# colopl/libpoporon

Measured on AMD Instinct MI355X. Metric: RS(255,223) codewords/s (encode; decode @ t=16 errs) and GB/s vs HBM peak, 1/2/4/8 GPU, higher is better.
Workload: dtype u8; 1 GPU; RS(255,223) round trip: encode + decode with 16 errors per codeword, 1048576 codewords per GPU (BASELINE configs[1]+[2]); codewords_per_gpu=1048576, layout=255-byte codeword rows, stride 255, code=poporon_config_rs_default (8, 0x11D, fcr 1, prim 1, 32 roots)

## Files before the change

### __graft_entry__.py

```python
import os
import subprocess
import sys
import time

ROOT = os.path.dirname(os.path.abspath(__file__))


def build() -> None:
    subprocess.check_call(["make", "-j8", "-C", os.path.join(ROOT, "libpoporon_amd")])
    subprocess.check_call(["make", "-C", os.path.join(ROOT, "testutil")])
    subprocess.check_call(["make", "-C", os.path.join(ROOT, "tests", "c")])
    subprocess.check_call(["make", "-C", os.path.join(ROOT, "oracle")])
    if ROOT not in sys.path:
        sys.path.insert(0, ROOT)
    import libpoporon_amd

    libpoporon_amd.load_library()


def _errors(rng, bad, span, nerr, exclude=None):
    import numpy as np
    n = bad.shape[0]
    key = rng.random((n, span))
    if exclude is not None:
        np.put_along_axis(key, exclude.astype(np.int64), -1.0, axis=1)
    nmax = int(np.max(nerr))
    pos = np.argsort(-key, axis=1)[:, :nmax]
    mag = rng.integers(1, 256, (n, nmax), dtype=np.uint8)
    if not np.isscalar(nerr):
        mag[np.arange(nmax)[None, :] >= np.asarray(nerr)[:, None]] = 0
    r = np.arange(n)[:, None]
    bad[r, pos] ^= mag
    return pos


def smoke() -> None:
    if ROOT not in sys.path:
        sys.path.insert(0, ROOT)
    import numpy as np
    import torch

    import libpoporon_amd as P
    from oracle import Oracle

    assert torch.cuda.is_available(), "smoke() needs cuda:0"
    torch.cuda.set_device(0)
    t0 = time.perf_counter()
    want_env = {"POPORON_AMD_DECODE_PATH": "split", "POPORON_AMD_DECODE_TAIL": "fused"}
    prev_env = {k: os.environ.get(k) for k in want_env}
    os.environ.update(want_env)
    try:
        rs = P.Poporon.default(device=0)
    finally:
        for k, v in prev_env.items():
            if v is None:
                del os.environ[k]
            else:
                os.environ[k] = v
    o = Oracle()
    th = min(16, os.cpu_count() or 1)
    rng = np.random.default_rng(0x5EED0001)
    n = 1 << 16
    K, NR = 223, 32
    s = torch.cuda.current_stream().cuda_stream

    data = rng.integers(0, 256, (n, K), dtype=np.uint8)
    cw = torch.zeros((n, 255), dtype=torch.uint8, device="cuda")
    cw[:, :K] = torch.from_numpy(data).cuda()
    rs.encode_batch_device(cw.data_ptr(), 255, cw.data_ptr() + K, 255, K, n, s)
    torch.cuda.synchronize()
    enc = cw.cpu().numpy()
    assert (enc[:, K:] == o.encode_batch(data, threads=th)).all(), "encode parity mismatch vs oracle"
    print(f"smoke encode: {n} messages, parity bit-exact vs oracle (rs_lfsr_k<ENCODE>)", flush=True)

    names = P.KERNEL_NAMES

    def decode(label, bad, expect, slots=None, cnt=None, kernels=""):
        d = torch.from_numpy(bad).cuda()
        ok = torch.zeros(n, dtype=torch.uint8, device="cuda")
        cor = torch.zeros(n, dtype=torch.uint8, device="cuda")
        kw = {}
        if slots is not None:
            sd = torch.from_numpy(np.ascontiguousarray(slots)).cuda()
            cd = torch.from_numpy(np.ascontiguousarray(cnt)).cuda()
            kw = dict(d_positions=sd.data_ptr(), positions_stride=slots.shape[1], d_counts=cd.data_ptr())
        rs.timing(True)
        rs.decode_batch_device(d.data_ptr(), 255, d.data_ptr() + K, 255, K, n, ok.data_ptr(), cor.data_ptr(),
                               stream=s, **kw)
        torch.cuda.synchronize()
        t = {k: rs.timing_read(k) for k in names}
        rs.timing(False)
        ran = {k for k, (ms, c) in t.items() if c}
        missing = [names[k] for k in expect if k not in ran]
        assert not missing, f"{label}: kernels that did not run: {missing}"
        assert P.KERNEL_CORRECT not in ran, f"{label}: the whole-batch general kernel ran instead of the split path"
        if slots is None:
            want = o.decode_batch(bad[:, :K], bad[:, K:], threads=th)
        else:
            want = o.decode_batch(bad[:, :K], bad[:, K:], slots.astype(np.uint32), cnt.astype(np.uint32), threads=th)
        out = d.cpu().numpy()
        gok, gcor = ok.cpu().numpy(), cor.cpu().numpy()
        assert (gok == want[0]).all(), f"{label}: ok differs at {np.nonzero(gok != want[0])[0][:8]}"
        assert (gcor == want[1]).all(), f"{label}: corrected_num differs at {np.nonzero(gcor != want[1])[0][:8]}"
        diff = np.nonzero((out[:, :K] != want[2]).any(1) | (out[:, K:] != want[3]).any(1))[0]
        assert diff.size == 0, f"{label}: decoded bytes differ at codewords {diff[:8]}"
        print(f"smoke {label}: {n} codewords bit-exact vs oracle (bytes, ok, corrected_num); ok {int(gok.sum())}, "
              f"corrected {int(gcor.sum())}; ran {kernels or ', '.join(names[k] for k in sorted(ran))}", flush=True)
        return gok, gcor, out

    bad = enc.copy()
    _errors(rng, bad, 255, 16)
    gok, gcor, out = decode("decode16", bad, (P.KERNEL_REMAINDER, P.KERNEL_BM, P.KERNEL_CHIEN, P.KERNEL_APPLY,
                                              P.KERNEL_LIST),
                            kernels="rs_lfsr_k<SYNDROME>, rs_bm_k, rs_chien_k, rs_forney_apply_k, "
                                    "rs_wave_k (list, empty)")
    assert gok.all() and (gcor == 16).all() and (out == enc).all()

    bad = enc.copy()
    slots = np.sort(np.argsort(rng.random((n, K)), axis=1)[:, :NR], axis=1).astype(np.uint8)
    bad[np.arange(n)[:, None], slots] ^= rng.integers(1, 256, (n, NR), dtype=np.uint8)
    cnt = np.full(n, NR, np.uint8)
    gok, gcor, out = decode("erasure32", bad, (P.KERNEL_REMAINDER, P.KERNEL_ERASURE, P.KERNEL_APPLY), slots, cnt,
                            kernels="rs_lfsr_k<SYNDROME>, rs_era_bp_k, rs_apply_k<32>")
    assert gok.all() and (gcor == NR).all() and (out == enc).all()

    bad = enc.copy()
    era = np.argsort(rng.random((n, K)), axis=1)[:, :16]
    slots = rng.integers(0, 255, (n, NR)).astype(np.uint8)
    slots[:, :16] = era
    bad[np.arange(n)[:, None], era] ^= rng.integers(1, 256, (n, 16), dtype=np.uint8)
    _errors(rng, bad, 255, 8, exclude=era)
    cnt = np.full(n, 16, np.uint8)
    decode("errata16e8", bad, (P.KERNEL_REMAINDER, P.KERNEL_ERASURE, P.KERNEL_BM, P.KERNEL_CHIEN, P.KERNEL_FORNEY,
                               P.KERNEL_APPLY, P.KERNEL_LIST), slots, cnt,
           kernels="rs_lfsr_k<SYNDROME>, rs_era_bp_k (hand-off), rs_ebm_k, rs_chien32_k, rs_forney32_k, "
                   "rs_wave_k (list), rs_apply_k<32>")

    bad = enc.copy()
    ne = np.minimum(rng.binomial(255, 0.045, n), 24)
    _errors(rng, bad, 255, ne)
    gok, _, _ = decode("mixed", bad, (P.KERNEL_REMAINDER, P.KERNEL_BM, P.KERNEL_CHIEN, P.KERNEL_APPLY, P.KERNEL_LIST),
                       kernels="rs_lfsr_k<SYNDROME>, rs_bm_k, rs_chien_k, rs_forney_apply_k, "
                               "rs_wave_k (list: L > 16 / deg != L, one wave per codeword)")
    assert (ne > 16).sum() > n // 50 and (gok == 0).sum() > 0

    for c in range(8):
        par = rs.encode(data[c])
        assert (par == enc[c, K:]).all(), "poporon_encode mismatch"
        b = enc[c].copy()
        _errors(rng, b[None, :], 255, 16 + (c & 1) * 2)
        got = rs.decode(b[:K], b[K:])
        want = o.decode(b[:K], b[K:])
        assert got[0] == want[0] and got[1] == want[1] and (got[2] == want[2]).all() and (got[3] == want[3]).all()
    print("smoke single calls: 8 x poporon_encode + poporon_decode (16 / 18 errors) bit-exact vs oracle "
          "(the single-call server rs_serve_k: enc1_body / dec1_body)", flush=True)
    ld = P.Ldpc(32, P.LDPC_RATE_1_2, P.LDPC_RANDOM, 3, False, True, True, max_iterations=20, device=0)
    msg = rng.integers(0, 256, (64, 32), dtype=np.uint8)
    ed, ep = ld.encode_batch(msg)
    assert not ld.check_batch(ed, ep).any(), "LDPC: encoded rows are not clean"
    rx = np.concatenate([ed, ep], axis=1)
    rx[np.arange(64), rng.integers(0, 32, 64)] ^= 0x80
    rx[np.arange(64), rng.integers(32, 64, 64)] ^= 0x01
    assert ld.check_batch(rx[:, :32], rx[:, 32:]).all(), "LDPC: flipped rows are not dirty"
    lok, lit, ldat, _ = ld.decode_batch(rx[:, :32], rx[:, 32:])
    won = lok == 1
    assert won.sum() >= 60 and (lit[won] >= 1).all() and (ldat[won] == msg[won]).all(), "LDPC: 2 flips not corrected"
    assert (ldat[~won] == rx[~won, :32]).all() and (lit[~won] == 20).all(), "LDPC: a failed row was rewritten"
    print(f"smoke ldpc: 64 rows of block 32 rate 1/2 (outer + inner interleaver) encoded, 2 bits flipped, decoded "
          f"({int(won.sum())} ok) in {int(lit.min())}..{int(lit.max())} iterations (ldpc_encode_k, ldpc_check_k, ldpc_decode_k)",
          flush=True)
    print(f"smoke ok ({time.perf_counter() - t0:.1f} s)", flush=True)


if __name__ == "__main__":
    build()
# ... 3 lines not shown
```

### libpoporon_amd/csrc/api.cpp

```cpp
#include <hip/hip_runtime.h>

#include <algorithm>
#include <atomic>
#include <chrono>
#include <cstdarg>
#include <cstdio>
#include <cstdlib>
#include <cstring>
#include <mutex>
#include <new>
#include <string>
#include <thread>
#include <vector>

#include "poporon.h"
#include "poporon_amd.h"
#include "rs_device.h"
#include "rs_generic.h"
#include "bch_device.h"
#include "ldpc_device.h"
#include "ldpc_graph.h"

#ifndef POPORON_BUILDTIME
#define POPORON_BUILDTIME 1
// ... 482 lines not shown
                    const uint64_t e = (uint64_t)(nr - 1 - m) * p.prim * (p.fcr + i);
                    rowb[i] = gmul(v << (4 * n), (uint32_t)(e % 255));
                }
                memcpy(&t.synt[((m * 2 + n) * 2 + 0) * 16 + v], rowb, 16);
                memcpy(&t.synt[((m * 2 + n) * 2 + 1) * 16 + v], rowb + 16, 16);
            }
        }
    }
    for (uint32_t j = 1; j <= 32; j++) {
        for (uint32_t e = 0; e < 256; e++) {
            uint8_t rowb[16];
            for (uint32_t b = 0; b < 16; b++)
                rowb[b] = e == 255 ? 0 : (uint8_t)gf->log2exp[(e + j * b) % 255];
            memcpy(&t.chien[(j - 1) * 256 + e], rowb, 16);
        }
    }
    uint32_t *gfa = reinterpret_cast<uint32_t *>(t.gfa);
    for (uint32_t x = 0; x < 512; x++)
        for (uint32_t r = 0; r < 32; r++) {
            const uint32_t la = x < 256u ? (x ? (uint32_t)t.log[x] * 128u + 4u * r + 1u : 128u * RS_Z0 + 4u * r) : 0u;
            gfa[x * 32 + r] = ((uint32_t)t.exp2[x] << 8) | (la << 16);
        }
    uint32_t *gfc = reinterpret_cast<uint32_t *>(t.gfc);
    for (uint32_t x = 0; x < 512; x++)
        for (uint32_t r = 0; r < 32; r++) {
            const uint32_t v = x & 255u;
            gfc[x * 32 + r] = ((uint32_t)t.exp2[x] << 8) | ((v ? (uint32_t)t.log[v] * 128u : 0xFFFFu) << 16);
        }
    const char *fv = getenv("POPORON_AMD_FORCE_VERIFY");
    p.force_verify = (fv && fv[0] == '1') ? 1u : 0u;
    const char *dp = getenv("POPORON_AMD_DECODE_PATH");
    h->decode_path = !dp ? 0 : !strcmp(dp, "split") ? 1 : !strcmp(dp, "single") ? 2 : !strcmp(dp, "wave") ? 3 : 0;
    const char *dt = getenv("POPORON_AMD_DECODE_TAIL");
    h->decode_tail = dt && !strcmp(dt, "split") ? 1 : dt && !strcmp(dt, "fused") ? 0 : h->decode_path == 1 ? 1 : 0;
}

static bool params_generic(const poporon_t *h)
{
    const poporon_rs_t *rs = h->rs;
    const uint32_t m = rs->gf->symbol_size, nn = rs->gf->field_size;
    return m >= 2 && m <= 8 && rs->num_roots >= 1 && rs->num_roots < nn && rs->primitive_element != 0;
}

static void build_generic(poporon_t *h)
{
    const poporon_rs_t *rs = h->rs;
    const poporon_gf_t *gf = rs->gf;
    RsGenTables &t = h->gen_tab;
    const uint32_t nn = gf->field_size;
    memset(&t, 0, sizeof(t));
    for (uint32_t i = 0; i < 256; i++) {
        t.alog[i] = i <= nn ? (uint8_t)gf->log2exp[i] : 0;
        t.log[i] = i <= nn ? (uint8_t)gf->exp2log[i] : (uint8_t)nn;
    }
    for (uint32_t i = 0; i <= rs->num_roots; i++)
        t.gen[i] = (uint8_t)rs->generator_polynomial[i];
    for (uint32_t fb = 0; fb < 256; fb++) {
        const uint32_t v = fb & nn;
        for (uint32_t i = 0; i < rs->num_roots && v != 0; i++)
            t.lrow[fb * 256 + i] = (uint8_t)gf->log2exp[gf_mod(
                gf, (uint16_t)(gf->exp2log[v] + rs->generator_polynomial[rs->num_roots - 1 - i]))];
    }
    {
        const uint32_t nr = rs->num_roots;
        const uint16_t *g = rs->generator_polynomial;
        memset(t.encq, 0xff, sizeof(t.encq));
        std::vector<uint8_t> reg(nr, 0);
// ... 1001 lines not shown
    bool shared = false;
    RsSplitWs ws = {};
};

static bool ws_acquire(poporon_t *h, uint8_t *rem, size_t rem_cap, size_t count, hipStream_t s, DecodeWs &w)
{
    w.shared = !rem;
    if (w.shared) {
        if (!ensure_rem(h, count) || !rem_acquire(h->gpu, s))
            return false;
        rem = h->gpu.rem;
        rem_cap = h->gpu.rem_cap;
    }
    w.rem = rem;
    w.ws = rs_ws_carve(rem, rem_cap ? rem_cap : count);
    return true;
}

static bool ws_release(poporon_t *h, const DecodeWs &w, hipStream_t s) { return !w.shared || rem_release(h->gpu, s); }

static hipError_t launch_list_nr(poporon_t *h, const DecodeCall &c, const RsSplitWs &ws)
{
    GpuCtx &g = h->gpu;
    const RsGenParams gp = gen_params(h, c.size);
    const size_t xs = c.ext_syn ? c.ext_stride : 0, es = c.pos8 ? c.pos_stride : 0;
    const uint8_t *cnt = c.pos8 ? c.cnt : nullptr;
    if (h->gen_path == 1)
        return rsg_decode_list(g.gtab, &gp, c.data, c.ds, c.par, c.ps, c.count, ws.list, ws.nlist, c.ext_syn, xs,
                               c.pos8, es, cnt, c.ok, c.corrected, g.num_cu, c.s);
    return rsgw_decode(g.gtab, &gp, c.data, c.ds, c.par, c.ps, c.count, c.ext_syn, xs, c.pos8, nullptr, es, cnt, c.ok,
                       c.corrected, ws.list, ws.nlist, nullptr, 0u, g.num_cu, c.s);
}

static bool launch_split(poporon_t *h, const DecodeCall &c)
{
    GpuCtx &g = h->gpu;
    hipStream_t s = c.s;
    const uint32_t npar = h->rs->num_roots, size = (uint32_t)c.size;
    const bool nr = npar < RS_NR;
    const RsCorrParams prm = corr_params(h, c.size);
    DecodeWs w;
    if (!ws_acquire(h, c.rem, c.rem_cap, c.count, s, w))
        return false;
    const RsSplitWs &ws = w.ws;
    STAGE(g, POPORON_AMD_KERNEL_REMAINDER, s,
          c.ext_syn ? rsk_ext_syn(g.tab, c.ext_syn, c.ext_stride, c.count, npar, ws.syn, ws.list, ws.nlist, s)
          : nr      ? rsk_syndrome_reset_nr(g.tab, c.data, c.ds, c.par, c.ps, size, c.count, ws.syn, ws.nlist, npar,
                                            g.num_cu, s)
                    : rsk_syndrome_reset(g.tab, c.data, c.ds, c.par, c.ps, size, c.count, ws.syn, ws.nlist, g.num_cu,
                                         s));
    STAGE(g, POPORON_AMD_KERNEL_BM, s,
          nr ? rsk_bm_nr(g.tab, &ws, c.count, npar, c.ok, c.corrected, g.num_cu, s)
             : rsk_bm(g.tab, &ws, c.count, c.ok, c.corrected, g.num_cu, s));
    STAGE(g, POPORON_AMD_KERNEL_CHIEN, s, rsk_chien(g.tab, &prm, &ws, c.count, c.ok, c.corrected, g.num_cu, s));
    if (h->decode_tail == 0) {
        STAGE(g, POPORON_AMD_KERNEL_APPLY, s,
              rsk_forney_apply(g.tab, &prm, &ws, c.data, c.ds, c.par, c.ps, c.count, npar, c.ok, c.corrected, g.num_cu,
                               s));
    } else {
        STAGE(g, POPORON_AMD_KERNEL_FORNEY, s,
              rsk_forney(g.tab, &prm, &ws, c.data, c.ds, c.par, c.ps, c.count, c.ok, c.corrected, g.num_cu, s));
        STAGE(g, POPORON_AMD_KERNEL_APPLY, s,
              nr ? rsk_apply_nr(&prm, &ws, c.data, c.ds, c.par, c.ps, c.count, npar, s)
                 : rsk_apply(&prm, &ws, c.data, c.ds, c.par, c.ps, c.count, s));
    }
    STAGE(g, POPORON_AMD_KERNEL_LIST, s,
          nr ? launch_list_nr(h, c, ws)
             : rsk_wave(g.tab, &prm, c.data, c.ds, c.par, c.ps, c.count, ws.list, ws.nlist,
                        c.ext_syn ? nullptr : ws.syn, c.ext_syn, c.ext_syn ? c.ext_stride : 0, nullptr, nullptr, 0,
                        nullptr, c.ok, c.corrected, g.num_cu, s));
    return ws_release(h, w, s);
}

static bool launch_errata(poporon_t *h, const DecodeCall &c, bool era_first, bool errata)
{
    GpuCtx &g = h->gpu;
    hipStream_t s = c.s;
    const uint32_t npar = h->rs->num_roots, size = (uint32_t)c.size;
    const bool nr = npar < RS_NR;
    const uint32_t only_pend = era_first ? 1u : 0u;
    const RsCorrParams prm = corr_params(h, c.size);
    DecodeWs w;
    if (!ws_acquire(h, c.rem, c.rem_cap, c.count, s, w))
        return false;
    const RsSplitWs &ws = w.ws;
    STAGE(g, POPORON_AMD_KERNEL_REMAINDER, s,
          nr ? rsk_syndrome_reset_nr(g.tab, c.data, c.ds, c.par, c.ps, size, c.count, ws.syn, ws.nlist, npar, g.num_cu,
                                     s)
// ... 1802 lines not shown
```

### libpoporon_amd/csrc/rs_device.h

```cpp
#ifndef POPORON_AMD_RS_DEVICE_H
#define POPORON_AMD_RS_DEVICE_H

#include <stddef.h>
#include <stdint.h>

#include <hip/hip_ext.h>
#include <hip/hip_runtime.h>

struct RsLaunchTimer {
    hipEvent_t start, stop;
    int n;
};
extern thread_local RsLaunchTimer rs_launch_timer;
#define RS_LAUNCH(K, G, B, SH, S, ...)                                                                    \
    do {                                                                                                 \
        if (rs_launch_timer.stop)                                                                        \
            hipExtLaunchKernelGGL(K, G, B, SH, S, rs_launch_timer.n++ ? nullptr : rs_launch_timer.start, \
                                  rs_launch_timer.stop, 0u, __VA_ARGS__);                                \
        else                                                                                             \
            hipLaunchKernelGGL(K, G, B, SH, S, __VA_ARGS__);                                             \
    } while (0)

#define RS_NR 32
#define RS_A0 255u
// ... 119 lines not shown

hipError_t rsk_check(const RsDevTables *tab, const uint8_t *data, size_t dstride, const uint8_t *parity, size_t pstride,
                     uint32_t size, size_t count, uint8_t *flag, int num_cu, hipStream_t stream);
hipError_t rsk_ext_syn(const RsDevTables *tab, const uint16_t *ext, size_t ext_stride, size_t count, uint32_t npar,
                       uint8_t *syn, uint32_t *list, uint32_t *nlist, hipStream_t stream);
hipError_t rsk_syn_log_nr(const RsDevTables *tab, const uint8_t *syn, size_t count, uint16_t *out, size_t stride,
                          uint8_t *flag, uint32_t npar, hipStream_t stream);
hipError_t rsk_check_nr(const RsDevTables *tab, const uint8_t *data, size_t dstride, const uint8_t *parity,
                        size_t pstride, uint32_t size, size_t count, uint8_t *flag, uint32_t npar, int num_cu,
                        hipStream_t stream);

hipError_t rsk_correct(const RsDevTables *tab, const RsCorrParams *prm, uint8_t *data, size_t dstride, uint8_t *parity,
                       size_t pstride, size_t count, const uint8_t *syn, const uint16_t *syn16, size_t syn16_stride,
                       const uint8_t *pos8,
                       const uint32_t *pos32, size_t pos_stride, const uint8_t *cnt, uint8_t *ok, uint8_t *corrected,
                       int num_cu, hipStream_t stream);

hipError_t rsk_correct_list(const RsDevTables *tab, const RsCorrParams *prm, uint8_t *data, size_t dstride,
                            uint8_t *parity, size_t pstride, size_t count, const uint8_t *syn, const uint32_t *list,
                            const uint32_t *list_n, uint8_t *ok, uint8_t *corrected, int num_cu, hipStream_t stream);

hipError_t rsk_bm(const RsDevTables *tab, const RsSplitWs *ws, size_t count, uint8_t *ok, uint8_t *corrected,
                  int num_cu, hipStream_t stream);
hipError_t rsk_chien(const RsDevTables *tab, const RsCorrParams *prm, const RsSplitWs *ws, size_t count, uint8_t *ok,
                     uint8_t *corrected, int num_cu, hipStream_t stream);
hipError_t rsk_forney(const RsDevTables *tab, const RsCorrParams *prm, const RsSplitWs *ws, uint8_t *data,
                      size_t dstride, uint8_t *parity, size_t pstride, size_t count, uint8_t *ok, uint8_t *corrected,
                      int num_cu, hipStream_t stream);
hipError_t rsk_apply(const RsCorrParams *prm, const RsSplitWs *ws, uint8_t *data, size_t dstride, uint8_t *parity,
                     size_t pstride, size_t count, hipStream_t stream);
hipError_t rsk_forney_apply(const RsDevTables *tab, const RsCorrParams *prm, const RsSplitWs *ws, uint8_t *data,
                            size_t dstride, uint8_t *parity, size_t pstride, size_t count, uint32_t npar, uint8_t *ok,
                            uint8_t *corrected, int num_cu, hipStream_t stream);

hipError_t rsk_syndrome_reset_nr(const RsDevTables *tab, const uint8_t *data, size_t dstride, const uint8_t *parity,
                                 size_t pstride, uint32_t size, size_t count, uint8_t *syn, uint32_t *reset,
                                 uint32_t npar, int num_cu, hipStream_t stream);
hipError_t rsk_bm_nr(const RsDevTables *tab, const RsSplitWs *ws, size_t count, uint32_t npar, uint8_t *ok,
                     uint8_t *corrected, int num_cu, hipStream_t stream);
hipError_t rsk_apply_nr(const RsCorrParams *prm, const RsSplitWs *ws, uint8_t *data, size_t dstride, uint8_t *parity,
                        size_t pstride, size_t count, uint32_t npar, hipStream_t stream);
hipError_t rsk_ebm_nr(const RsDevTables *tab, const RsCorrParams *prm, const RsSplitWs *ws, const uint8_t *pos8,
                      size_t pos_stride, const uint8_t *cnt, size_t count, uint8_t *ok, uint8_t *corrected,
                      uint32_t npar, int num_cu, hipStream_t stream);
hipError_t rsk_forney32_nr(const RsDevTables *tab, const RsCorrParams *prm, const RsSplitWs *ws, const uint8_t *pos8,
                           size_t pos_stride, size_t count, uint8_t *ok, uint8_t *corrected, uint32_t npar,
                           int num_cu, hipStream_t stream);
hipError_t rsk_apply_era_nr(const RsCorrParams *prm, const uint8_t *meta, const uint8_t *rec, uint8_t *data,
                            size_t dstride, uint8_t *parity, size_t pstride, size_t count, uint32_t npar,
                            hipStream_t stream);

hipError_t rsk_correct_era_rec(const RsDevTables *tab, const RsCorrParams *prm, size_t count, const uint8_t *syn,
                               const uint8_t *pos8, const uint32_t *pos32, size_t pos_stride, const uint8_t *cnt,
                               uint8_t *ok, uint8_t *corrected, uint8_t *rec, uint8_t *meta, int num_cu,
                               hipStream_t stream);
hipError_t rsk_era(const RsDevTables *tab, const RsCorrParams *prm, const RsSplitWs *ws, const uint8_t *pos8,
                   size_t pos_stride, const uint8_t *cnt, size_t count, uint8_t *ok, uint8_t *corrected, uint32_t pend,
                   int num_cu, hipStream_t stream);
hipError_t rsk_correct_era_list(const RsDevTables *tab, const RsCorrParams *prm, size_t count, const uint8_t *syn,
                                const uint8_t *pos8, size_t pos_stride, const uint8_t *cnt, uint8_t *ok,
                                uint8_t *corrected, uint8_t *rec, uint8_t *meta, const uint32_t *list,
                                const uint32_t *list_n, int num_cu, hipStream_t stream);
hipError_t rsk_apply_era(const RsCorrParams *prm, const uint8_t *meta, const uint8_t *rec, uint8_t *data,
                         size_t dstride, uint8_t *parity, size_t pstride, size_t count, hipStream_t stream);

hipError_t rsk_ebm(const RsDevTables *tab, const RsCorrParams *prm, const RsSplitWs *ws, const uint8_t *pos8,
// ... 33 lines not shown
```

### libpoporon_amd/csrc/rs_fast.hip

```cpp
#include <hip/hip_runtime.h>

#include <type_traits>

#include "rs_device.h"
#include "rs_gfa.h"
#include "rs_lane.h"

#define FWG 1024
#define NL 17
#define BWG 512
#define BM_WAVES 4

#define FAST_ROUNDS 8
static int fast_grid(size_t count, int num_cu)
{
    const size_t need = (count + FWG - 1) / FWG;
    const size_t g = FAST_ROUNDS * 2u * (size_t)(num_cu > 0 ? num_cu : 256);
    return (int)(need < g ? (need ? need : 1) : g);
}


template <bool NRG>
__global__ __launch_bounds__(BWG, BM_WAVES) void rs_bm_k(const RsDevTables *__restrict__ T, const uint8_t *__restrict__ syn,
                                                   size_t count, uint8_t *__restrict__ lamo, uint8_t *__restrict__ omo,
// ... 655 lines not shown
        }
        __builtin_amdgcn_fence(__ATOMIC_RELEASE, "wavefront");
        __builtin_amdgcn_wave_barrier();
        __builtin_amdgcn_fence(__ATOMIC_ACQUIRE, "wavefront");
#pragma unroll
        for (uint32_t k = 0; k < 16; ++k) {
            const uint32_t c = lane + 64u * k;
            if (c < ABLK) {
                const uint4 v = im[c];
                __builtin_nontemporal_store(lds_u32x4_t{v.x, v.y, v.z, v.w}, reinterpret_cast<lds_u32x4_t *>(dst + c));
            }
        }
    } else if (fast) {
        uint8_t *cdata = data + cw * dstride, *cpar = parity + cw * pstride;
#pragma unroll
        for (int n = 0; n < NC; ++n) {
            const uint32_t mg = (mw[n >> 2] >> (8 * (n & 3))) & 0xffu;
            const uint32_t p = (pw[n >> 2] >> (8 * (n & 3))) & 0xffu;
            if (mg && p < lim) {
                uint8_t *d = p < size ? cdata + p : cpar + (p - size);
                *d = (uint8_t)(*d ^ mg);
            }
        }
    }
}


#define FAWG 1024
#define FAQ 255u
#ifndef FA_PRE
#define FA_PRE 2
#endif

template <bool P11>
__device__ __forceinline__ uint32_t forney_lane(const GfA gf, const uint32_t fcr, const uint32_t iprim,
                                                const int32_t pad, uint32_t deg, const uint4 o4, const uint4 l4,
                                                const uint32_t (&rl)[4], uint32_t (&posp)[4], uint32_t (&magp)[4])
{
    constexpr bool fcr1 = P11, iprim1 = P11;
    constexpr int R = FORNEY_R;
    const uint32_t mp = 255u * 128u + gf.pofs;
    const uint32_t ow[4] = {o4.x, o4.y, o4.z, o4.w}, lw[4] = {l4.x, l4.y, l4.z, l4.w};
    const uint32_t dtop = deg ? (deg - 1u) & ~1u : 0u;
    uint32_t opu[16], lod[8];
#pragma unroll
    for (int m = 0; m < 16; ++m)
        opu[m] = gf.afrom((ow[m >> 2] >> (8 * (m & 3))) & 0xffu);
#pragma unroll
    for (int h = 0; h < 8; ++h)
        lod[h] = (uint32_t)(2 * h) <= dtop ? gf.afrom((lw[(2 * h) >> 2] >> (8 * ((2 * h) & 3))) & 0xffu) : gf.az();
    const uint32_t degmax = wave_max(deg);
    uint32_t fixed = 0;
#pragma unroll
    for (int k = 0; k < 4; ++k)
        posp[k] = magp[k] = 0;
#pragma unroll
    for (int n0 = 0; n0 < 16; n0 += R) {
        if ((uint32_t)n0 >= degmax)
            continue;
        uint32_t ir[R], si[R], s[R], num[R], den[R], nh[R], dh[R];
#pragma unroll
        for (int t = 0; t < R; ++t) {
            ir[t] = root_point((rl[(n0 + t) >> 2] >> (8 * ((n0 + t) & 3))) & 0xffu);
            si[t] = 128u * (ir[t] == 255u ? 0u : ir[t]);
            s[t] = num[t] = den[t] = nh[t] = dh[t] = 0;
        }
#pragma unroll
        for (int b = 0; b < 8; ++b) {
// ... 117 lines not shown
                            atomicXor(stw + (a >> 2), mg << (8u * (a & 3u)));
                        }
                    }
                }
                __builtin_amdgcn_fence(__ATOMIC_RELEASE, "wavefront");
                __builtin_amdgcn_wave_barrier();
                __builtin_amdgcn_fence(__ATOMIC_ACQUIRE, "wavefront");
#pragma unroll
                for (uint32_t k = 0; k < 4; ++k)
                    if (lane + 64u * k < FAQ) {
                        const uint4 r = st[lane + 64u * k];
                        __builtin_nontemporal_store(lds_u32x4_t{r.x, r.y, r.z, r.w}, rows + FAQ * q + lane + 64u * k);
                    }
                __builtin_amdgcn_fence(__ATOMIC_RELEASE, "wavefront");
                __builtin_amdgcn_wave_barrier();
                __builtin_amdgcn_fence(__ATOMIC_ACQUIRE, "wavefront");
            }
        } else if (fast) {
            uint8_t *cdata = data + cw * dstride, *cpar = parity + cw * pstride;
#pragma unroll
            for (int n = 0; n < 16; ++n) {
                const uint32_t mg = (magp[n >> 2] >> (8 * (n & 3))) & 0xffu;
                const uint32_t p = (posp[n >> 2] >> (8 * (n & 3))) & 0xffu;
                if (mg && p < lim) {
                    uint8_t *d = p < P.size ? cdata + p : cpar + (p - P.size);
                    *d = (uint8_t)(*d ^ mg);
                }
            }
        }
    }
}


extern "C" hipError_t rsk_bm(const RsDevTables *tab, const RsSplitWs *ws, size_t count, uint8_t *ok,
                             uint8_t *corrected, int num_cu, hipStream_t stream)
{
    if (count == 0)
        return hipSuccess;
    const size_t need = (count + BWG - 1) / BWG,
                 res = FAST_ROUNDS * (size_t)(num_cu > 0 ? num_cu : 256) * (BM_WAVES * 256 / BWG);
    RS_LAUNCH(rs_bm_k<false>, dim3((uint32_t)(need < res ? need : res)), dim3(BWG), 0, stream, tab, ws->syn, count,
              ws->lam, ws->om, ws->meta, ws->list, ws->nlist, ok, corrected, (uint32_t)RS_NR);
    return hipGetLastError();
}

extern "C" hipError_t rsk_bm_nr(const RsDevTables *tab, const RsSplitWs *ws, size_t count, uint32_t npar, uint8_t *ok,
                                uint8_t *corrected, int num_cu, hipStream_t stream)
{
    if (count == 0)
        return hipSuccess;
    const size_t need = (count + BWG - 1) / BWG,
                 res = FAST_ROUNDS * (size_t)(num_cu > 0 ? num_cu : 256) * (BM_WAVES * 256 / BWG);
    RS_LAUNCH(rs_bm_k<true>, dim3((uint32_t)(need < res ? need : res)), dim3(BWG), 0, stream, tab, ws->syn, count,
              ws->lam, ws->om, ws->meta, ws->list, ws->nlist, ok, corrected, npar);
    return hipGetLastError();
}

extern "C" hipError_t rsk_chien(const RsDevTables *tab, const RsCorrParams *prm, const RsSplitWs *ws, size_t count,
                                uint8_t *ok, uint8_t *corrected, int num_cu, hipStream_t stream)
{
    if (count == 0)
        return hipSuccess;
    RS_LAUNCH(rs_chien_k, dim3(fast_grid(count, num_cu)), dim3(FWG), 0, stream, tab, *prm, count, ws->lam,
                       ws->meta, ws->roots, ok, corrected);
    return hipGetLastError();
}
// ... 4 lines not shown
{
    if (count == 0)
        return hipSuccess;
    const size_t need = (count + F2WG - 1) / F2WG, cap = FAST_ROUNDS * 2u * (size_t)(num_cu > 0 ? num_cu : 256);
    const dim3 grid((uint32_t)(need < cap ? need : cap));
    if (prm->fcr == 1u && prm->iprim == 1u)
        RS_LAUNCH(rs_forney_k<true>, grid, dim3(F2WG), 0, stream, tab, *prm, data, dstride, parity, pstride, count,
                  ws->lam, ws->om, ws->roots, ws->meta, ok, corrected);
    else
        RS_LAUNCH(rs_forney_k<false>, grid, dim3(F2WG), 0, stream, tab, *prm, data, dstride, parity, pstride, count,
                  ws->lam, ws->om, ws->roots, ws->meta, ok, corrected);
    return hipGetLastError();
}

extern "C" hipError_t rsk_forney_apply(const RsDevTables *tab, const RsCorrParams *prm, const RsSplitWs *ws,
                                       uint8_t *data, size_t dstride, uint8_t *parity, size_t pstride, size_t count,
                                       uint32_t npar, uint8_t *ok, uint8_t *corrected, int num_cu, hipStream_t stream)
{
    if (count == 0)
        return hipSuccess;
    const uint32_t wire = prm->size + npar == 255u && dstride == 255u && pstride == 255u &&
                          parity == data + prm->size && (reinterpret_cast<uintptr_t>(data) & 15u) == 0u;
    const size_t need = (count + FAWG - 1) / FAWG, cap = (size_t)(num_cu > 0 ? num_cu : 256);
    const dim3 grid((uint32_t)(need < cap ? need : cap));
    if (prm->fcr == 1u && prm->iprim == 1u)
        RS_LAUNCH(rs_forney_apply_k<true>, grid, dim3(FAWG), 0, stream, tab, *prm, data, dstride, parity, pstride,
                  count, ws->lam, ws->om, ws->roots, ws->meta, ok, corrected, wire, npar);
    else
        RS_LAUNCH(rs_forney_apply_k<false>, grid, dim3(FAWG), 0, stream, tab, *prm, data, dstride, parity, pstride,
                  count, ws->lam, ws->om, ws->roots, ws->meta, ok, corrected, wire, npar);
    return hipGetLastError();
}

template <int NC>
static hipError_t apply_launch(const RsCorrParams *prm, const uint8_t *meta, const uint8_t *rec, uint8_t *data,
                               size_t dstride, uint8_t *parity, size_t pstride, size_t count, hipStream_t stream,
                               uint32_t npar = RS_NR)
{
    if (count == 0)
        return hipSuccess;
    const uint32_t wire = prm->size + npar == 255u && dstride == 255u && pstride == 255u &&
                          parity == data + prm->size && (reinterpret_cast<uintptr_t>(data) & 15u) == 0u;
    const size_t waves = (count + 63) / 64;
    RS_LAUNCH(rs_apply_k<NC>, dim3((uint32_t)((waves + AWG / 64 - 1) / (AWG / 64))), dim3(AWG), 0, stream,
                       meta, rec, data, dstride, parity, pstride, prm->size, count, wire, npar);
    return hipGetLastError();
}

extern "C" hipError_t rsk_apply(const RsCorrParams *prm, const RsSplitWs *ws, uint8_t *data, size_t dstride,
                                uint8_t *parity, size_t pstride, size_t count, hipStream_t stream)
{
    return apply_launch<16>(prm, ws->meta, ws->roots, data, dstride, parity, pstride, count, stream);
}

extern "C" hipError_t rsk_apply_nr(const RsCorrParams *prm, const RsSplitWs *ws, uint8_t *data, size_t dstride,
                                   uint8_t *parity, size_t pstride, size_t count, uint32_t npar, hipStream_t stream)
{
    return apply_launch<16>(prm, ws->meta, ws->roots, data, dstride, parity, pstride, count, stream, npar);
}

extern "C" hipError_t rsk_apply_era_nr(const RsCorrParams *prm, const uint8_t *meta, const uint8_t *rec, uint8_t *data,
                                       size_t dstride, uint8_t *parity, size_t pstride, size_t count, uint32_t npar,
                                       hipStream_t stream)
{
    return apply_launch<32>(prm, meta, rec, data, dstride, parity, pstride, count, stream, npar);
}
// ... 20 lines not shown
```

Baseline: 2.008 billion codewords/s.

## Fuse Chien search into Forney-apply kernel for large split-path decode batches

Adds rs_search_apply_k, which runs the Chien root search per codeword from LDS-resident tables and immediately feeds the roots to Forney and the in-place correction. It also software-pipelines the next wave's search against the current wave's staged row writes. This removes the separate rs_chien_k launch and the round trip of roots through global memory. By default the fused path is chosen when the batch exceeds 1024 codewords per CU, so it applies to the benchmark size. In exchange it uses the full 160 KB of LDS per 1024-thread block, which limits occupancy, and the kernel has significantly more complex control flow.

```diff
diff --git a/__graft_entry__.py b/__graft_entry__.py
--- a/__graft_entry__.py
+++ b/__graft_entry__.py
@@ -46,7 +46,7 @@
     assert torch.cuda.is_available(), "smoke() needs cuda:0"
     torch.cuda.set_device(0)
     t0 = time.perf_counter()
-    want_env = {"POPORON_AMD_DECODE_PATH": "split", "POPORON_AMD_DECODE_TAIL": "fused"}
+    want_env = {"POPORON_AMD_DECODE_PATH": "split", "POPORON_AMD_DECODE_TAIL": "search"}
     prev_env = {k: os.environ.get(k) for k in want_env}
     os.environ.update(want_env)
     try:
@@ -110,10 +110,8 @@
 
     bad = enc.copy()
     _errors(rng, bad, 255, 16)
-    gok, gcor, out = decode("decode16", bad, (P.KERNEL_REMAINDER, P.KERNEL_BM, P.KERNEL_CHIEN, P.KERNEL_APPLY,
-                                              P.KERNEL_LIST),
-                            kernels="rs_lfsr_k<SYNDROME>, rs_bm_k, rs_chien_k, rs_forney_apply_k, "
-                                    "rs_wave_k (list, empty)")
+    gok, gcor, out = decode("decode16", bad, (P.KERNEL_REMAINDER, P.KERNEL_BM, P.KERNEL_APPLY, P.KERNEL_LIST),
+                            kernels="rs_lfsr_k<SYNDROME>, rs_bm_k, rs_search_apply_k, rs_wave_k (list, empty)")
     assert gok.all() and (gcor == 16).all() and (out == enc).all()
 
     bad = enc.copy()
@@ -139,8 +137,8 @@
     bad = enc.copy()
     ne = np.minimum(rng.binomial(255, 0.045, n), 24)
     _errors(rng, bad, 255, ne)
-    gok, _, _ = decode("mixed", bad, (P.KERNEL_REMAINDER, P.KERNEL_BM, P.KERNEL_CHIEN, P.KERNEL_APPLY, P.KERNEL_LIST),
-                       kernels="rs_lfsr_k<SYNDROME>, rs_bm_k, rs_chien_k, rs_forney_apply_k, "
+    gok, _, _ = decode("mixed", bad, (P.KERNEL_REMAINDER, P.KERNEL_BM, P.KERNEL_APPLY, P.KERNEL_LIST),
+                       kernels="rs_lfsr_k<SYNDROME>, rs_bm_k, rs_search_apply_k, "
                                "rs_wave_k (list: L > 16 / deg != L, one wave per codeword)")
     assert (ne > 16).sum() > n // 50 and (gok == 0).sum() > 0
 
diff --git a/libpoporon_amd/csrc/api.cpp b/libpoporon_amd/csrc/api.cpp
--- a/libpoporon_amd/csrc/api.cpp
+++ b/libpoporon_amd/csrc/api.cpp
@@ -538,7 +538,11 @@
     const char *dp = getenv("POPORON_AMD_DECODE_PATH");
     h->decode_path = !dp ? 0 : !strcmp(dp, "split") ? 1 : !strcmp(dp, "single") ? 2 : !strcmp(dp, "wave") ? 3 : 0;
     const char *dt = getenv("POPORON_AMD_DECODE_TAIL");
-    h->decode_tail = dt && !strcmp(dt, "split") ? 1 : dt && !strcmp(dt, "fused") ? 0 : h->decode_path == 1 ? 1 : 0;
+    h->decode_tail = dt && !strcmp(dt, "split")    ? 1
+                     : dt && !strcmp(dt, "fused")  ? 0
+                     : dt && !strcmp(dt, "search") ? 2
+                     : h->decode_path == 1         ? 1
+                                                   : 3;
 }
 
 static bool params_generic(const poporon_t *h)
@@ -1606,6 +1610,14 @@
                        c.corrected, ws.list, ws.nlist, nullptr, 0u, g.num_cu, c.s);
 }
 
+static int split_tail(const poporon_t *h, size_t count)
+{
+    if (h->decode_tail != 3)
+        return h->decode_tail;
+    const size_t cus = (size_t)(h->gpu.num_cu > 0 ? h->gpu.num_cu : 256);
+    return count > cus * 1024u ? 2 : 0;
+}
+
 static bool launch_split(poporon_t *h, const DecodeCall &c)
 {
     GpuCtx &g = h->gpu;
@@ -1626,8 +1638,14 @@
     STAGE(g, POPORON_AMD_KERNEL_BM, s,
           nr ? rsk_bm_nr(g.tab, &ws, c.count, npar, c.ok, c.corrected, g.num_cu, s)
              : rsk_bm(g.tab, &ws, c.count, c.ok, c.corrected, g.num_cu, s));
-    STAGE(g, POPORON_AMD_KERNEL_CHIEN, s, rsk_chien(g.tab, &prm, &ws, c.count, c.ok, c.corrected, g.num_cu, s));
-    if (h->decode_tail == 0) {
+    const int tail = split_tail(h, c.count);
+    if (tail != 2)
+        STAGE(g, POPORON_AMD_KERNEL_CHIEN, s, rsk_chien(g.tab, &prm, &ws, c.count, c.ok, c.corrected, g.num_cu, s));
+    if (tail == 2) {
+        STAGE(g, POPORON_AMD_KERNEL_APPLY, s,
+              rsk_search_apply(g.tab, &prm, &ws, c.data, c.ds, c.par, c.ps, c.count, npar, c.ok, c.corrected, g.num_cu,
+                               s));
+    } else if (tail == 0) {
         STAGE(g, POPORON_AMD_KERNEL_APPLY, s,
               rsk_forney_apply(g.tab, &prm, &ws, c.data, c.ds, c.par, c.ps, c.count, npar, c.ok, c.corrected, g.num_cu,
                                s));
diff --git a/libpoporon_amd/csrc/rs_device.h b/libpoporon_amd/csrc/rs_device.h
--- a/libpoporon_amd/csrc/rs_device.h
+++ b/libpoporon_amd/csrc/rs_device.h
@@ -175,6 +175,9 @@
 hipError_t rsk_forney_apply(const RsDevTables *tab, const RsCorrParams *prm, const RsSplitWs *ws, uint8_t *data,
                             size_t dstride, uint8_t *parity, size_t pstride, size_t count, uint32_t npar, uint8_t *ok,
                             uint8_t *corrected, int num_cu, hipStream_t stream);
+hipError_t rsk_search_apply(const RsDevTables *tab, const RsCorrParams *prm, const RsSplitWs *ws, uint8_t *data,
+                            size_t dstride, uint8_t *parity, size_t pstride, size_t count, uint32_t npar, uint8_t *ok,
+                            uint8_t *corrected, int num_cu, hipStream_t stream);
 
 hipError_t rsk_syndrome_reset_nr(const RsDevTables *tab, const uint8_t *data, size_t dstride, const uint8_t *parity,
                                  size_t pstride, uint32_t size, size_t count, uint8_t *syn, uint32_t *reset,
diff --git a/libpoporon_amd/csrc/rs_fast.hip b/libpoporon_amd/csrc/rs_fast.hip
--- a/libpoporon_amd/csrc/rs_fast.hip
+++ b/libpoporon_amd/csrc/rs_fast.hip
@@ -711,8 +711,8 @@
 #define FA_PRE 2
 #endif
 
-template <bool P11>
-__device__ __forceinline__ uint32_t forney_lane(const GfA gf, const uint32_t fcr, const uint32_t iprim,
+template <bool P11, class G = GfA>
+__device__ __forceinline__ uint32_t forney_lane(const G gf, const uint32_t fcr, const uint32_t iprim,
                                                 const int32_t pad, uint32_t deg, const uint4 o4, const uint4 l4,
                                                 const uint32_t (&rl)[4], uint32_t (&posp)[4], uint32_t (&magp)[4])
 {
@@ -896,6 +896,312 @@
 }
 
 
+#define SAWG 1024
+#define SA_CH 0u
+#define SA_GF (255u * 256u)
+#define SA_ST (SA_GF + 65536u)
+#define SA_WIN 2048u
+#define SA_Z (SA_ST + (SAWG / 64) * SA_WIN)
+#define SA_END (SA_Z + 256u)
+
+template <uint32_t B>
+struct GfAt : GfA {
+    __device__ __forceinline__ uint32_t expa(uint32_t a) const { return lds8(a + B); }
+    __device__ __forceinline__ uint32_t loga(uint32_t v) const { return lds16(pofs + 1u + (v << 7) + B); }
+    __device__ __forceinline__ uint32_t logs(uint32_t v) const { return loga(v) - pofs; }
+    __device__ __forceinline__ uint32_t exp(uint32_t l) const { return lds8(pofs + (l << 7) + B); }
+};
+
+__device__ __forceinline__ void wave_sync_lds()
+{
+    __builtin_amdgcn_fence(__ATOMIC_RELEASE, "wavefront");
+    __builtin_amdgcn_wave_barrier();
+    __builtin_amdgcn_fence(__ATOMIC_ACQUIRE, "wavefront");
+}
+
+__device__ __forceinline__ bool search_lane(const RsCorrParams &P, const bool fast, const uint32_t deg, const uint4 l4,
+                                            const uint32_t lp0, const uint32_t cw, uint8_t *__restrict__ meta,
+                                            uint8_t *__restrict__ ok, uint8_t *__restrict__ corrected,
+                                            uint32_t (&rl)[4])
+{
+    constexpr uint32_t WRAP = 255u * 256u;
+    uint32_t lr = threadIdx.x & 15u;
+    asm volatile("" : "+v"(lr));
+    uint32_t D[4] = {l4.x, l4.y, l4.z, l4.w};
+    uint32_t E[4];
+#pragma unroll
+    for (int k = 0; k < 4; ++k)
+        E[k] = (lr & 4u) ? D[(k + 1) & 3] : D[k];
+#pragma unroll
+    for (int k = 0; k < 4; ++k)
+        D[k] = (lr & 8u) ? E[(k + 2) & 3] : E[k];
+    uint32_t R[4];
+#pragma unroll
+    for (int k = 0; k < 4; ++k)
+        R[k] = __builtin_amdgcn_alignbyte(D[(k + 1) & 3], D[k], lr & 3u);
+    uint32_t oz = 0;
+    asm volatile("" : "+v"(oz));
+    const uint32_t zrow = oz + SA_Z, wrap = oz + WRAP;
+    uint32_t A[16], inc[16];
+#pragma unroll
+    for (int k = 0; k < 16; ++k) {
+        const uint32_t jm = ((uint32_t)k + lr) & 15u;
+        const uint32_t e = (R[k >> 2] >> (8 * (k & 3))) & 0xffu;
+        A[k] = (e == 255u ? zrow : SA_CH + (e << 8)) + (jm << 4);
+        inc[k] = e == 255u ? wrap : (jm == 15u ? 256u : (jm + 1u) << 12);
+    }
+    *(__attribute__((address_space(3))) lds_u32x4_t *)(size_t)lp0 = lds_u32x4_t{oz, oz, oz, oz};
+    uint32_t lp = lp0;
+    uint32_t cnt = 0, z0 = 0;
+    auto push = [&](uint32_t v) __attribute__((always_inline)) {
+        lds_st8(lp, v);
+        lp += 1u;
+    };
+#pragma unroll 1
+    for (int w = 0; w < 8; ++w) {
+        uint32_t word = 0;
+#pragma unroll
+        for (int h = 0; h < 2; ++h) {
+            uint32_t acc[4] = {0x01010101u, 0x01010101u, 0x01010101u, 0x01010101u};
+#pragma unroll
+            for (int k = 0; k < 16; k += 2) {
+                const lds_u32x4_t r1 = lds128(A[k]), r2 = lds128(A[k + 1]);
+                A[k] = chien_step<WRAP>(A[k], inc[k]);
+                A[k + 1] = chien_step<WRAP>(A[k + 1], inc[k + 1]);
+                acc[0] = xor3(acc[0], r1.x, r2.x);
+                acc[1] = xor3(acc[1], r1.y, r2.y);
+                acc[2] = xor3(acc[2], r1.z, r2.z);
+                acc[3] = xor3(acc[3], r1.w, r2.w);
+            }
+#pragma unroll
+            for (int d = 0; d < 4; ++d)
+                word = __builtin_amdgcn_bitop3_b32(word, zero80(acc[d]) >> (d + 4 * h), 0u, 0xF0 | 0xCC);
+        }
+        if (w == 7)
+            word &= ~(1u << 24);
+        if (w == 0) {
+            z0 = (word >> 7) & 1u;
+            word &= ~0x80u;
+        }
+        cnt += __popc(word);
+        const uint32_t wb = 32u * (uint32_t)w;
+        while (word != 0u) {
+            const uint32_t b = __builtin_ctz(word);
+            word &= word - 1u;
+            push(wb | b);
+        }
+    }
+    if (z0)
+        push(248u);
+    cnt += z0;
+    const lds_u32x4_t l4r = lds128(lp0);
+    rl[0] = l4r.x, rl[1] = l4r.y, rl[2] = l4r.z, rl[3] = l4r.w;
+    bool good = cnt == deg;
+    if (P.pad > 0) {
+        bool low = false;
+#pragma unroll
+        for (int n = 0; n < 16; ++n) {
+            const uint32_t i = root_point((rl[n >> 2] >> (8 * (n & 3))) & 0xffu);
+            low |= (uint32_t)n < cnt && (int32_t)((i * P.iprim + 254u) % 255u) < P.pad;
+        }
+        good = good && !low;
+    }
+    if (fast && !good) {
+        ok[cw] = 0;
+        if (corrected)
+            corrected[cw] = 0;
+        meta[cw] = (uint8_t)(RS_ST_DONE << 5);
+    }
+    return fast && good;
+}
+
+template <bool P11>
+__global__ __launch_bounds__(SAWG, SAWG / 256) void rs_search_apply_k(
+    const RsDevTables *__restrict__ T, RsCorrParams P, uint8_t *data, size_t dstride, uint8_t *parity, size_t pstride,
+    size_t count, const uint8_t *__restrict__ lam, const uint8_t *__restrict__ om, uint8_t *__restrict__ meta,
+    uint8_t *__restrict__ ok, uint8_t *__restrict__ corrected, uint32_t wire, uint32_t npar)
+{
+    static_assert(SA_END == 163840u && SA_GF <= 65535u, "the whole LDS; the GF image inside the DS offset field");
+    __shared__ uint4 lds[SA_END / 16];
+    {
+        constexpr uint32_t NCH = 255u * 16u;
+        uint4 v[4];
+#pragma unroll
+        for (int k = 0; k < 4; ++k) {
+            const uint32_t t = min(threadIdx.x + k * SAWG, NCH - 1u);
+            v[k] = T->chien[(t & 15u) * 256u + (t >> 4)];
+        }
+#pragma unroll
+        for (int k = 0; k < 4; ++k)
+            if (threadIdx.x + k * SAWG < NCH)
+                lds[SA_CH / 16 + threadIdx.x + k * SAWG] = v[k];
+        if (threadIdx.x < 16u)
+            lds[SA_Z / 16 + threadIdx.x] = make_uint4(0, 0, 0, 0);
+    }
+    fill_gfa<SAWG>(reinterpret_cast<uint32_t *>(lds + SA_GF / 16), T);
+    __syncthreads();
+    const GfAt<SA_GF> gf{4u * (threadIdx.x & 31u) + 1u};
+    const uint32_t lane = threadIdx.x & 63u;
+    const uint32_t wv = __builtin_amdgcn_readfirstlane(threadIdx.x >> 6);
+    uint4 *st = lds + SA_ST / 16 + wv * (SA_WIN / 16);
+    uint32_t *stw = reinterpret_cast<uint32_t *>(st);
+    const uint32_t lp0 = SA_ST + wv * SA_WIN + 16u * lane;
+    const uint32_t lim = P.size + npar;
+    const uint4 none = make_uint4(0xFFFFFFFFu, 0xFFFFFFFFu, 0xFFFFFFFFu, 0xFFFFFFFFu);
+    const lds_u32x4_t *img = reinterpret_cast<const lds_u32x4_t *>(T->gfa);
+    const uint32_t c3 = min(lane + 192u, FAQ - 1u);
+
+    const uint32_t rofs = (lane & 15u) * 255u;
+    auto stage_quarter = [&](const uint32_t q, const lds_u32x4_t (&vq)[4], lds_u32x4_t *rows, const uint32_t pq,
+                             const uint32_t mq) __attribute__((always_inline)) {
+#pragma unroll
+        for (uint32_t wn = 0; wn < 2; ++wn) {
+#pragma unroll
+            for (uint32_t j = 0; j < 2; ++j) {
+                const uint32_t k = 2u * wn + j;
+                if (lane + 64u * k < FAQ)
+                    st[lane + 64u * j] = make_uint4(vq[k].x, vq[k].y, vq[k].z, vq[k].w);
+            }
+            wave_sync_lds();
+#pragma unroll
+            for (int n = 0; n < 4; ++n) {
+                const uint32_t mg = (mq >> (8 * n)) & 0xffu;
+                const uint32_t p = (pq >> (8 * n)) & 0xffu;
+                const uint32_t a = rofs + p;
+                if (mg && p < lim && (a >> 11) == wn)
+                    atomicXor(stw + ((a & (SA_WIN - 1u)) >> 2), mg << (8u * (a & 3u)));
+            }
+            wave_sync_lds();
+#pragma unroll
+            for (uint32_t j = 0; j < 2; ++j) {
+                const uint32_t k = 2u * wn + j;
+                if (lane + 64u * k < FAQ) {
+                    const uint4 r = st[lane + 64u * j];
+                    __builtin_nontemporal_store(lds_u32x4_t{r.x, r.y, r.z, r.w}, rows + FAQ * q + lane + 64u * k);
+                }
+            }
+            wave_sync_lds();
+        }
+    };
+
+    const uint32_t nb = (uint32_t)((count + SAWG - 1) / SAWG), cq = (uint32_t)(count >> 6), cr = (uint32_t)count & 63u;
+    auto rows_of = [&](const uint32_t wi) __attribute__((always_inline)) {
+        return wi < cq ? 64u : wi == cq ? cr : 0u;
+    };
+
+    uint32_t b = blockIdx.x;
+    uint32_t wi = (nb - 1u - b) * (SAWG / 64) + wv, nrow = rows_of(wi);
+    uint32_t deg;
+    bool fast;
+    uint32_t rl[4] = {0, 0, 0, 0};
+    {
+        const size_t wbase = (size_t)wi * 64u;
+        const uint32_t mt = lane < nrow ? meta[wbase + lane] : 0u;
+        fast = (mt >> 5) == RS_ST_FAST;
+        deg = fast ? (mt & 31u) : 0u;
+        if (__ballot(fast) != 0ull) {
+            const uint4 l4 = fast ? reinterpret_cast<const uint4 *>(lam)[wbase + lane] : none;
+            fast = search_lane(P, fast, deg, l4, lp0, lane, meta + wbase, ok + wbase,
+                               corrected ? corrected + wbase : nullptr, rl);
+            wave_sync_lds();
+            deg = fast ? deg : 0u;
+        }
+    }
+
+    for (;;) {
+        const size_t wbase = (size_t)wi * 64u;
+        const uint32_t bn = b + gridDim.x;
+        const bool more = bn < nb;
+        const bool block = wire && nrow == 64u && __ballot(fast) != 0ull;
+        const uint32_t nwi = more ? (nb - 1u - bn) * (SAWG / 64) + wv : 0u, nnrow = more ? rows_of(nwi) : 0u;
+        const size_t nwbase = nnrow ? (size_t)nwi * 64u : 0u, cbase = nrow ? wbase : 0u;
+        const uint32_t nl = lane < nnrow ? lane : 0u, cl = lane < nrow ? lane : 0u;
+        uint4 o4 = (reinterpret_cast<const uint4 *>(om) + cbase)[cl];
+        uint4 l4 = (reinterpret_cast<const uint4 *>(lam) + cbase)[cl];
+        uint32_t nmt = (meta + nwbase)[nl];
+        lds_u32x4_t *rows = reinterpret_cast<lds_u32x4_t *>(data + wbase * 255u);
+        const lds_u32x4_t *pre = block ? rows : img;
+        lds_u32x4_t v[2][4];
+#pragma unroll
+        for (int q = 0; q < 2; ++q)
+#pragma unroll
+            for (uint32_t k = 0; k < 4; ++k)
+                v[q][k] = __builtin_nontemporal_load(pre + FAQ * q + (k < 3 ? lane + 64u * k : c3));
+        __builtin_amdgcn_sched_barrier(0);
+        if (!fast)
+            o4 = l4 = none;
+        uint32_t posp[4], magp[4];
+        const uint32_t fixed = forney_lane<P11>(gf, P.fcr, P.iprim, P.pad, deg, o4, l4, rl, posp, magp);
+        if (fast) {
+            (ok + wbase)[lane] = 1;
+            if (corrected)
+                (corrected + wbase)[lane] = (uint8_t)fixed;
+        }
+        uint32_t pq[4] = {0, 0, 0, 0}, mq[4] = {0, 0, 0, 0};
+        if (block) {
+#pragma unroll
+            for (uint32_t q = 0; q < 4; ++q) {
+                const int src = (int)(4u * (16u * q + (lane & 15u)));
+#pragma unroll
+                for (uint32_t k = 0; k < 4; ++k) {
+                    const uint32_t pk = (uint32_t)__builtin_amdgcn_ds_bpermute(src, (int)posp[k]);
+                    const uint32_t mk = (uint32_t)__builtin_amdgcn_ds_bpermute(src, (int)magp[k]);
+                    pq[q] = (lane >> 4) == k ? pk : pq[q];
+                    mq[q] = (lane >> 4) == k ? mk : mq[q];
+                }
+            }
+        } else if (fast) {
+            const size_t cw = wbase + lane;
+            uint8_t *cdata = data + cw * dstride, *cpar = parity + cw * pstride;
+#pragma unroll
+            for (int n = 0; n < 16; ++n) {
+                const uint32_t mg = (magp[n >> 2] >> (8 * (n & 3))) & 0xffu;
+                const uint32_t p = (posp[n >> 2] >> (8 * (n & 3))) & 0xffu;
+                if (mg && p < lim) {
+                    uint8_t *d = p < P.size ? cdata + p : cpar + (p - P.size);
+                    *d = (uint8_t)(*d ^ mg);
+                }
+            }
+        }
+        nmt = lane < nnrow ? nmt : 0u;
+        bool nfast = (nmt >> 5) == RS_ST_FAST;
+        const uint32_t ndeg = nfast ? (nmt & 31u) : 0u;
+        uint4 nl4 = (reinterpret_cast<const uint4 *>(lam) + nwbase)[nl];
+        __builtin_amdgcn_sched_barrier(0);
+        if (block) {
+            stage_quarter(0u, v[0], rows, pq[0], mq[0]);
+            stage_quarter(1u, v[1], rows, pq[1], mq[1]);
+        }
+        const lds_u32x4_t *pre2 = block ? rows + 2u * FAQ : img;
+#pragma unroll
+        for (int q = 0; q < 2; ++q)
+#pragma unroll
+            for (uint32_t k = 0; k < 4; ++k)
+                v[q][k] = __builtin_nontemporal_load(pre2 + FAQ * q + (k < 3 ? lane + 64u * k : c3));
+        __builtin_amdgcn_sched_barrier(0);
+        if (!nfast)
+            nl4 = none;
+        if (__ballot(nfast) != 0ull) {
+            nfast = search_lane(P, nfast, ndeg, nl4, lp0, lane, meta + nwbase, ok + nwbase,
+                                corrected ? corrected + nwbase : nullptr, rl);
+            wave_sync_lds();
+        }
+        __builtin_amdgcn_sched_barrier(0);
+        if (block) {
+            stage_quarter(2u, v[0], rows, pq[2], mq[2]);
+            stage_quarter(3u, v[1], rows, pq[3], mq[3]);
+        }
+        if (!more)
+            break;
+        b = bn;
+        wi = nwi;
+        nrow = nnrow;
+        fast = nfast;
+        deg = nfast ? ndeg : 0u;
+    }
+}
+
+
 extern "C" hipError_t rsk_bm(const RsDevTables *tab, const RsSplitWs *ws, size_t count, uint8_t *ok,
                              uint8_t *corrected, int num_cu, hipStream_t stream)
 {
@@ -966,6 +1272,27 @@
     return hipGetLastError();
 }
 
+extern "C" hipError_t rsk_search_apply(const RsDevTables *tab, const RsCorrParams *prm, const RsSplitWs *ws,
+                                       uint8_t *data, size_t dstride, uint8_t *parity, size_t pstride, size_t count,
+                                       uint32_t npar, uint8_t *ok, uint8_t *corrected, int num_cu, hipStream_t stream)
+{
+    if (count == 0)
+        return hipSuccess;
+    if (count >> 38)
+        return hipErrorInvalidValue;
+    const uint32_t wire = prm->size + npar == 255u && dstride == 255u && pstride == 255u &&
+                          parity == data + prm->size && (reinterpret_cast<uintptr_t>(data) & 15u) == 0u;
+    const size_t need = (count + SAWG - 1) / SAWG, cap = (size_t)(num_cu > 0 ? num_cu : 256);
+    const dim3 grid((uint32_t)(need < cap ? need : cap));
+    if (prm->fcr == 1u && prm->iprim == 1u)
+        RS_LAUNCH(rs_search_apply_k<true>, grid, dim3(SAWG), 0, stream, tab, *prm, data, dstride, parity, pstride,
+                  count, ws->lam, ws->om, ws->meta, ok, corrected, wire, npar);
+    else
+        RS_LAUNCH(rs_search_apply_k<false>, grid, dim3(SAWG), 0, stream, tab, *prm, data, dstride, parity, pstride,
+                  count, ws->lam, ws->om, ws->meta, ok, corrected, wire, npar);
+    return hipGetLastError();
+}
+
 template <int NC>
 static hipError_t apply_launch(const RsCorrParams *prm, const uint8_t *meta, const uint8_t *rec, uint8_t *data,
                                size_t dstride, uint8_t *parity, size_t pstride, size_t count, hipStream_t stream,
```

Measured after the change: 2.158 billion codewords/s (median of 6 runs). 1.07x the previous value.
